# Sohojoe/ppo-dash

Measured on AMD Instinct MI355X. Metric: env-steps/sec (rollout+GAE+PPO update) at 4096 envs×128 steps, 1/2/4/8 MI355X, higher is better.
Workload: dtype f32

## Files before the change

ppo-dash_amd/csrc/conv1.hip:

```cpp
#include "conv_launch.h"
#include "conv1_fwd_body.h"
#include "conv1_paths.h"

namespace {
template <typename InT, class C_>
struct Conv1Fwd : C_ {
  using BCtx = typename C_::BCtx;
  const InT* obs; const int64_t* idx; long long row0; int C, M;
  const float* w; const float* bias; float* out;
  struct ACtx { const InT* base; bool ok; };
  __device__ ACtx a_ctx(int m, int) const {
    if (m >= M) return {obs, false};
    const int b = m / 400, pp = m - b * 400, oy = pp / 20, ox = pp - oy * 20;
    return {obs + obs_row(idx, row0, b) * (long long)(C * IMG2) + (oy * 4) * IMG + ox * 4, true};
  }
  using Raw = std::conditional_t<sizeof(InT) == 1, uint32_t, f32x4>;
  __device__ Raw a_load(const ACtx& c, int k) const {
    if (!c.ok) return Raw{};
    const int ch = k >> 6, ky = (k >> 3) & 7, kx = k & 7;
    return *reinterpret_cast<const Raw*>(c.base + ch * IMG2 + ky * IMG + kx);
  }
  __device__ BCtx b_ctx(int n, int) const { return {w + n * (C * 64), 0, n < 32}; }
  __device__ f32x4 b_load(const BCtx& c, int k) const {
    return c.ok ? *reinterpret_cast<const f32x4*>(c.p + k) : zero4();
  }
  __device__ void k_range(int, int& b, int& e) const { b = 0; e = C * 64; }
  __device__ void store(int m, int n, int, float v) const {
    if constexpr (sizeof(InT) == 1) v *= (1.0f / 255.0f);
    if (m < M) out[(size_t)m * 32 + n] = fmaxf(v + bias[n], 0.f);
  }
};

template <int C, bool MASK, int NPW = 3>
__global__ __launch_bounds__(512) void conv1_fwd_bf16x3_kernel(const uint8_t* __restrict__ obs,
                                                               const int64_t* __restrict__ idx, long long row0,
                                                               int B, const float* __restrict__ w,
                                                               const float* __restrict__ bias,
                                                               float* __restrict__ out,
                                                               uint16_t* __restrict__ mbits) {
  __shared__ __attribute__((aligned(16))) uint16_t img[2][C * C1S];
  conv1_fwd_bf16x3_body<C, MASK, NPW>(obs, idx, row0, B, w, bias, out, mbits, img);
}

template <int NPD = 3, int NW = 8, int TPW = 1>
__global__ __launch_bounds__(NW * 64) void conv1_wgrad_parts_kernel(const float* __restrict__ dz1,
                                                                const uint8_t* __restrict__ obs,
                                                                const int64_t* __restrict__ idx, long long row0,
                                                                int B, float* __restrict__ slab,
                                                                float* __restrict__ slab_bias, int dbg) {
  const bool no_mma = dbg & 1, no_put = dbg & 2, no_dma = dbg & 4;
  constexpr int C = 4, NPART = 5, ER = 20, SLOTS = 40, DZS = 88, MAXIMG = 512;
  constexpr int E_BF = C * ER * SLOTS * 4, DZ_BF = 32 * DZS, STG = E_BF + 3 * DZ_BF;
  constexpr int EPC = 105, EPIECE = 448, DPIECE = 640, RAWP = EPIECE + DPIECE;
  __shared__ __attribute__((aligned(16))) uint16_t L[2 * STG];
  __shared__ __attribute__((aligned(16))) uint4 RAW[3][RAWP];
  __shared__ long long rowtab[MAXIMG];
  __shared__ float bred[320];
  static_assert(NW == 8 || NW == 16, "8 or 16 waves");
  static_assert(TPW == 1 || (TPW == 2 && NW == 16), "two tiles per wave with 16 waves");
  constexpr int NT = NW * 64;
  const int tid = threadIdx.x, lane = tid & 63, wave = tid >> 6, l32 = lane & 31, h = lane >> 5;
  const int tile = TPW == 2 ? 2 * (wave & 3) : wave & 7, kh = TPW == 2 ? wave >> 2 : wave >> 3;
  const int G = gridDim.x;
  const int nimg = blockIdx.x < B ? (B - 1 - (int)blockIdx.x) / G + 1 : 0, nit = NPART * nimg;
  for (int k = tid; k < nimg; k += NT) rowtab[k] = obs_row(idx, row0, (int)blockIdx.x + k * G);
  int qoff[TPW][5][2];
#pragma unroll
  for (int t = 0; t < TPW; ++t) {
    const int tt = tile + t, bc = tt >> 1, bky = 4 * (tt & 1) + (l32 >> 3), bkx = l32 & 7;
#pragma unroll
    for (int ls = 0; ls < 5; ++ls)
#pragma unroll
      for (int j = 0; j < 2; ++j) {
        const int ql = 4 * ls + 2 * h + j, oyl = ql / 5, Q = ql - 5 * oyl;
        const int r = bc * ER + 4 * oyl + bky, item = r * 5 + Q;
        qoff[t][ls][j] = (r * SLOTS + Q * 8 + (bkx ^ ((item >> 1) & 7))) * 4;
      }
  }
  const int aoff = E_BF + l32 * DZS + 8 * h;
  const bool e_on = tid < 400, d_on = NW == 8 ? tid < 320 : tid >= 512 && tid < 832;
  const int eit = e_on ? tid : 0, dit = d_on ? tid - (NW == 8 ? 0 : 512) : 0;
  const int er = eit / 5, eQ = eit - 5 * er, ec = er / ER, eyr = er - ER * ec, ef = (eit >> 1) & 7;
  const int dco = dit & 31, doc = dit >> 5;
  float bacc = 0.f;
  auto dma = [&](int j) {
    if (no_dma) return;
    const int jj = j < nit ? j : nit - 1, k = jj / NPART, p = jj - NPART * k, b = (int)blockIdx.x + k * G;
    uint4* dst = RAW[jj % 3];
    if (wave < 7) {
      const int piece = min(64 * wave + lane, C * EPC - 1), c = piece / EPC, r = piece - EPC * c;
      const uint8_t* src = obs + rowtab[k] * (long long)(C * IMG2) + c * IMG2 + p * (16 * IMG) + 16 * r;
      __builtin_amdgcn_global_load_lds(reinterpret_cast<const void*>(src),
                                       reinterpret_cast<__attribute__((address_space(3))) void*>(
                                           reinterpret_cast<uintptr_t>(dst + 64 * wave)), 16, 0, 0);
    }
    const char* dsrc = reinterpret_cast<const char*>(dz1 + (size_t)b * 12800 + p * 80 * 32);
#pragma unroll
    for (int i = 0; i < (NW == 8 ? 2 : 1); ++i) {
      const int blk = NW == 8 ? wave + 8 * i : wave - 6;
      if (blk >= 0 && blk < DPIECE / 64)
        __builtin_amdgcn_global_load_lds(reinterpret_cast<const void*>(dsrc + 16 * (64 * blk + lane)),
                                         reinterpret_cast<__attribute__((address_space(3))) void*>(
                                             reinterpret_cast<uintptr_t>(dst + EPIECE + 64 * blk)), 16, 0, 0);
    }
  };
  auto put = [&](int j, int st) {
    if (no_put) return;
    const uint32_t* R = reinterpret_cast<const uint32_t*>(RAW[j % 3]);
    uint32_t ew[5];
    float dv[8];
    if (NW == 8 || e_on) {
#pragma unroll
      for (int q = 0; q < 5; ++q) ew[q] = R[(ec * 1680 + eyr * IMG + 16 * eQ) / 4 + q];
    }
    if (NW == 8 || d_on) {
#pragma unroll
      for (int q = 0; q < 8; ++q) dv[q] = __uint_as_float(R[4 * EPIECE + (8 * doc + q) * 32 + dco]);
    }
    uint16_t* S = L + st * STG;
    if (e_on) {
#pragma unroll
      for (int kx = 0; kx < 8; ++kx) {
        const int o = kx >> 2, sh = 8 * (kx & 3);
        float f[4];
// ... 115 lines not shown
#pragma unroll
      for (int t = 0; t < 2; ++t)
#pragma unroll
        for (int r = 0; r < 16; ++r) X[xo(tp, t, r)] = acc[t][r];
    }
    __syncthreads();
    if (kh == 0) {
#pragma unroll
      for (int t = 0; t < 2; ++t)
#pragma unroll
        for (int r = 0; r < 16; ++r) acc[t][r] += X[xo(tp, t, r)];
    }
  }
  float* out = slab + (size_t)blockIdx.x * 32 * 256;
  if (kh == 0) {
#pragma unroll
    for (int t = 0; t < TPW; ++t)
#pragma unroll
      for (int r = 0; r < 16; ++r) {
        const int co = (r & 3) + 8 * (r >> 2) + 4 * h, n = 32 * (tile + t) + l32;
        out[co * 256 + n] = acc[t][r];
      }
  }
  if (d_on) bred[dit] = bacc;
  __syncthreads();
  if (tid < 32) {
    float t = 0.f;
#pragma unroll
    for (int o = 0; o < 10; ++o) t += bred[32 * o + tid];
    slab_bias[(size_t)blockIdx.x * 32 + tid] = t;
  }
}

__global__ __launch_bounds__(256) void relu_bits_kernel(const float* __restrict__ a1, long long halves,
                                                        uint16_t* __restrict__ mbits) {
  for (long long i = (long long)blockIdx.x * 256 + threadIdx.x; i < halves; i += (long long)gridDim.x * 256) {
    const f32x4* p = reinterpret_cast<const f32x4*>(a1 + 16 * i);
    uint32_t m = 0;
#pragma unroll
    for (int q = 0; q < 4; ++q) {
      const f32x4 v = p[q];
#pragma unroll
      for (int e = 0; e < 4; ++e) m |= (v[e] > 0.f ? 1u : 0u) << (4 * q + e);
    }
    mbits[i] = (uint16_t)m;
  }
}

template <typename InT, class C_>
struct Conv1Wgrad : WgradBase<C_> {
  static_assert(400 % C_::BK == 0, "conv1 wgrad k-tiles must not straddle images");
  static constexpr bool B_TILE = true;
  const InT* obs; const int64_t* idx; long long row0; int C;
  struct BCtx { int off; bool ok; };
  struct TCtx { const InT* img; int r0; };
  using Raw = std::conditional_t<sizeof(InT) == 1, uint32_t, f32x4>;
  __device__ BCtx b_ctx(int n, int) const {
    const int ch = n >> 6, ky = (n >> 3) & 7, kx = n & 7;
    return {ch * IMG2 + ky * IMG + kx, n < C * 64};
  }
  __device__ TCtx tile(int k0) const {
    const int b = k0 / 400;
    return {obs + obs_row(idx, row0, b) * (long long)(C * IMG2), b * 400};
  }
  __device__ Raw b_load_t(const BCtx& c, const TCtx& t, int r) const {
    if (!c.ok || r >= this->R) return Raw{};
    const int pp = r - t.r0, oy = pp / 20, ox = pp - oy * 20;
    return *reinterpret_cast<const Raw*>(t.img + (oy * 4) * IMG + ox * 4 + c.off);
  }
};

using V32_0 = Cfg<256, 32, 4, 1, true, true>;
using CfgW32 = Cfg<32, 256, 1, 4, false, false, true>;

}

static int conv1_fwd_impl(const void* obs, int obs_is_u8, const int64_t* idx, long long row0, int C, int B,
                          const float* w1, const float* b1, float* out, uint16_t* mbits, void* stream) {
  PPO_REQUIRE(B >= 0 && C > 0, "ppo_conv1_fwd: B=%d C=%d", B, C);
  if (!mbits && B > 0 && B <= tune_small_b() && C <= 8)
    return small_conv1_fwd(obs, obs_is_u8, idx, row0, C, B, w1, b1, out, as_stream(stream));
  if (!obs_is_u8 && C == 4 && ((uintptr_t)obs & 15) == 0)
    return ppo_conv1_fwd_f32((const float*)obs, idx, row0, B, w1, b1, out, reinterpret_cast<uint32_t*>(mbits), stream);
  const bool img = obs_is_u8 && C == 4 && tune_key(TK_CONV1_FWD) == 0;
  if (mbits && !img) {
    const int rc = conv1_fwd_impl(obs, obs_is_u8, idx, row0, C, B, w1, b1, out, nullptr, stream);
    if (rc != 0 || B == 0) return rc;
    const long long halves = (long long)B * 800;
    const long long nb = (halves + 255) / 256;
    relu_bits_kernel<<<(unsigned)(nb < 8192 ? nb : 8192), 256, 0, as_stream(stream)>>>(out, halves, mbits);
    PPO_LAUNCH_CHECK("relu_bits_kernel");
    return 0;
  }
  const long long M = (long long)B * 400;
  const double fl = 2.0 * M * 32 * C * 64;
  if (img) {
    if (B == 0) return 0;
    const unsigned nb = img_grid(B);
    int slot;
    const bool prof = ppo_prof_begin("conv1_fwd_u8", as_stream(stream), &slot);
    const uint8_t* o8 = (const uint8_t*)obs;
    hipStream_t st = as_stream(stream);
    if (tune_products() == 1) {
      if (mbits) conv1_fwd_bf16x3_kernel<4, true, 1><<<nb, 512, 0, st>>>(o8, idx, row0, B, w1, b1, out, mbits);
      else conv1_fwd_bf16x3_kernel<4, false, 1><<<nb, 512, 0, st>>>(o8, idx, row0, B, w1, b1, out, nullptr);
    } else if (mbits) {
      conv1_fwd_bf16x3_kernel<4, true><<<nb, 512, 0, st>>>(o8, idx, row0, B, w1, b1, out, mbits);
    } else {
      conv1_fwd_bf16x3_kernel<4, false><<<nb, 512, 0, st>>>(o8, idx, row0, B, w1, b1, out, nullptr);
    }
    if (prof) ppo_prof_end(slot, st, fl);
    PPO_LAUNCH_CHECK("conv1_fwd_u8 (image-resident)");
    return 0;
  }
#define SETUP1(T_)                                                                                 \
  p.obs = (const T_*)obs; p.idx = idx; p.row0 = row0; p.C = C; p.M = (int)M; p.w = w1; p.bias = b1; p.out = out
  if (obs_is_u8) {
    Conv1Fwd<uint8_t, V32_0> p;
    SETUP1(uint8_t);
    return launch(p, M, 32, 1, as_stream(stream), "conv1_fwd_u8", fl);
  }
  Conv1Fwd<float, V32_0> p;
  SETUP1(float);
  return launch(p, M, 32, 1, as_stream(stream), "conv1_fwd_f32", fl);
#undef SETUP1
}

PPO_API int ppo_conv1_fwd(const void* obs, int obs_is_u8, const int64_t* idx, long long row0, int C, int B,
                          const float* w1, const float* b1, float* out, void* stream) {
  return conv1_fwd_impl(obs, obs_is_u8, idx, row0, C, B, w1, b1, out, nullptr, stream);
}

PPO_API int ppo_conv1_fwd_mask(const void* obs, int obs_is_u8, const int64_t* idx, long long row0, int C, int B,
                               const float* w1, const float* b1, float* out, uint32_t* mbits, void* stream) {
  PPO_REQUIRE(mbits != nullptr, "ppo_conv1_fwd_mask: null mask");
  return conv1_fwd_impl(obs, obs_is_u8, idx, row0, C, B, w1, b1, out, reinterpret_cast<uint16_t*>(mbits), stream);
}

PPO_API int ppo_conv1_wgrad(const float* dz1, const void* obs, int obs_is_u8, const int64_t* idx, long long row0,
                            int C, int B, int Z, float* slab, float* slab_bias, void* stream) {
  const long long R = (long long)B * 400;
  PPO_REQUIRE(R < 0x7fffffffLL, "ppo_conv1_wgrad: B too large");
  if (B <= 0 || Z <= 0) return 0;
  const double fl = 2.0 * R * 32 * C * 64;
  const int kw = tune_key(TK_CONV1_WGRAD), np = tune_products();
  if (obs_is_u8 && C == 4 && (kw == 5 || np == 1)) {
    if (B <= 0 || Z <= 0) return 0;
    PPO_REQUIRE((B + Z - 1) / Z <= 512, "ppo_conv1_wgrad: %d images over %d blocks (at most 512 per block)", B, Z);
    int slot;
    const bool prof = ppo_prof_begin("conv1_wgrad_u8", as_stream(stream), &slot);
    if (np == 1)
      conv1_wgrad_parts_kernel<1, 16, 2><<<Z, 1024, 0, as_stream(stream)>>>(dz1, (const uint8_t*)obs, idx, row0, B,
                                                                            slab, slab_bias, 0);
    else
      conv1_wgrad_parts_kernel<3, 16, 2><<<Z, 1024, 0, as_stream(stream)>>>(dz1, (const uint8_t*)obs, idx, row0, B,
                                                                            slab, slab_bias, tune_stagger() >> 4);
    if (prof) ppo_prof_end(slot, as_stream(stream), fl);
    PPO_LAUNCH_CHECK("conv1_wgrad_parts_kernel");
    return 0;
  }
  if (obs_is_u8 && C == 4)
    return kw >= 9
               ? conv1_wgrad_kw3(dz1, (const uint8_t*)obs, idx, row0, B, Z, slab, slab_bias, stream, kw == 10 ? 8 : 4)
               : conv1_wgrad_kw(dz1, (const uint8_t*)obs, idx, row0, B, Z, slab, slab_bias, stream);
  if (!obs_is_u8 && C == 4 && ((uintptr_t)obs & 15) == 0)
    return ppo_conv1_wgrad_f32(dz1, (const float*)obs, idx, row0, B, Z, slab, slab_bias, stream);
  if (obs_is_u8) {
    Conv1Wgrad<uint8_t, CfgW32> p;
    set_wgrad(p, dz1, 32, R, Z, slab, slab_bias, C * 64);
    p.obs = (const uint8_t*)obs; p.idx = idx; p.row0 = row0; p.C = C;
    return launch(p, 32, C * 64, Z, as_stream(stream), "conv1_wgrad_u8", fl);
  }
  Conv1Wgrad<float, CfgW32> p;
  set_wgrad(p, dz1, 32, R, Z, slab, slab_bias, C * 64);
  p.obs = (const float*)obs; p.idx = idx; p.row0 = row0; p.C = C;
  return launch(p, 32, C * 64, Z, as_stream(stream), "conv1_wgrad_f32", fl);
}
```

ppo-dash_amd/csrc/conv1_fwd_body.h:

```cpp
#pragma once
#include "igemm_x9.h"

namespace {

constexpr int IMG = 84, IMG2 = 84 * 84;
constexpr int C1S = 7104;
static_assert(C1S >= IMG2 && (C1S / 2) % 64 == 32, "conv1 stage channel stride");

template <int C, bool MASK, int NPW = 3>
__device__ __forceinline__ void conv1_fwd_bf16x3_body(const uint8_t* __restrict__ obs,
                                                      const int64_t* __restrict__ idx, long long row0, int B,
                                                      const float* __restrict__ w, const float* __restrict__ bias,
                                                      float* __restrict__ out, uint16_t* __restrict__ mbits,
                                                      uint16_t (*__restrict__ img)[C * C1S]) {
  constexpr int NPX = C * IMG2, CH = NPX / 16, K = C * 64, KS = K / 32, PER = (CH + 511) / 512;
  constexpr int CCH = IMG2 / 16;
  static_assert(IMG2 % 16 == 0 && C % 2 == 0, "16-pixel chunks, channel pairs");
  const int tid = threadIdx.x, lane = tid & 63, wave = tid >> 6;
  const int ct = wave & 1, rq = wave >> 1;
  const int i16 = lane & 15, g = lane >> 4;
  const int col = ct * 16 + i16;
  const float bv = bias[col];
  bf16x8 wf[3][KS];
#pragma unroll
// ... 27 lines not shown
        const uint32_t v[4] = {stage[j].x, stage[j].y, stage[j].z, stage[j].w};
        uint32_t o[8];
#pragma unroll
        for (int q = 0; q < 4; ++q) {
          const f32x4 f = to_f32x4(v[q]);
          o[2 * q] = __builtin_amdgcn_perm(__float_as_uint(f[1]), __float_as_uint(f[0]), 0x07060302u);
          o[2 * q + 1] = __builtin_amdgcn_perm(__float_as_uint(f[3]), __float_as_uint(f[2]), 0x07060302u);
        }
        const int ch = c / CCH;
        uint4* d = reinterpret_cast<uint4*>(img[buf] + ch * C1S + 16 * (c - ch * CCH));
        d[0] = uint4{o[0], o[1], o[2], o[3]};
        d[1] = uint4{o[4], o[5], o[6], o[7]};
      }
    }
  };
  const int G = gridDim.x;
  int b = blockIdx.x, cur = 0;
  if (b < B) {
    fetch(b);
    put(0);
    if (b + G < B) fetch(b + G);
  }
  __syncthreads();
  for (; b < B; b += G) {
    if (b + G < B) put(cur ^ 1);
    if (b + 2 * G < B) fetch(b + 2 * G);
    auto tiles = [&](auto ntc) __attribute__((always_inline)) {
      constexpr int NTL = decltype(ntc)::value;
      const uint16_t* I = img[cur];
      f32x4 acc[NTL];
#pragma unroll
      for (int t = 0; t < NTL; ++t) acc[t] = zero4();
      int pix[NTL];
#pragma unroll
      for (int t = 0; t < NTL; ++t) {
        const int row = (rq + 4 * t) * 16 + i16, oy = row / 20, ox = row - oy * 20;
        pix[t] = (g & 1) * C1S + (g >> 1) * IMG + oy * (4 * IMG) + ox * 4;
      }
#pragma unroll
      for (int s = 0; s < KS; ++s) {
        const uint16_t* Is = I + 2 * (s >> 2) * C1S + 2 * (s & 3) * IMG;
        bf16x8 a[NTL];
#pragma unroll
        for (int t = 0; t < NTL; ++t) {
          typedef uint32_t u32x2 __attribute__((ext_vector_type(2)));
          const volatile __attribute__((address_space(3))) u32x2* p2 =
              (const volatile __attribute__((address_space(3))) u32x2*)(Is + pix[t]);
          const u32x2 lo = p2[0], hi = p2[1];
          a[t] = __builtin_bit_cast(bf16x8, uint4{lo.x, lo.y, hi.x, hi.y});
        }
#pragma unroll
        for (int part = 0; part < NPW; ++part)
#pragma unroll
          for (int t = 0; t < NTL; ++t)
            acc[t] = __builtin_amdgcn_mfma_f32_16x16x32_bf16(a[t], wf[part][s], acc[t], 0, 0, 0);
      }
      float* o = out + (size_t)b * (400 * 32) + col;
#pragma unroll
      for (int t = 0; t < NTL; ++t) {
          const int rt = rq + 4 * t;
          uint64_t bal[4];
#pragma unroll
          for (int r = 0; r < 4; ++r) {
            const float v = fmaxf(acc[t][r] * (1.0f / 255.0f) + bv, 0.f);
            o[(rt * 16 + 4 * g + r) * 32] = v;
            if constexpr (MASK) bal[r] = __builtin_amdgcn_ballot_w64(v > 0.f);
          }
          if constexpr (MASK) {
            if (lane < 16) {
              const int r = lane & 3, gg = lane >> 2;
              const uint64_t bsel = r == 0 ? bal[0] : r == 1 ? bal[1] : r == 2 ? bal[2] : bal[3];
              mbits[((size_t)b * 400 + rt * 16 + lane) * 2 + ct] = (uint16_t)(bsel >> (16 * gg));
            }
          }
        }
    };
    if (rq == 0) tiles(std::integral_constant<int, 7>{});
    else tiles(std::integral_constant<int, 6>{});
    __syncthreads();
    cur ^= 1;
  }
}

constexpr int C1F_LDS = 2 * 4 * C1S * 2;

}
```

ppo-dash_amd/csrc/trunk.hip:

```cpp
#include "conv_launch.h"
#include "conv1_fwd_body.h"
#include "conv2_fwd_body.h"
#include "conv3_fwd_body.h"

namespace {

constexpr int max_of(int a, int b) { return a > b ? a : b; }
constexpr int TRUNK_LDS = max_of(max_of(C1F_LDS, C2F_LDS), max_of(C3C_LDS0, C3L_LDS));
static_assert(C2L_LDS <= TRUNK_LDS, "the trunk's conv2 lone tiles in the shared LDS");

__device__ __forceinline__ void trunk_phase_sync() {
  asm volatile("s_waitcnt vmcnt(0)" ::: "memory");
  __syncthreads();
  __builtin_amdgcn_fence(__ATOMIC_ACQUIRE, "agent");
}

template <int NP>
__global__ __launch_bounds__(512) void trunk_fwd_kernel(const uint8_t* __restrict__ obs, const int64_t* __restrict__ idx,
                                                       long long row0, int B, const float* __restrict__ w1,
                                                       const float* __restrict__ b1, float* __restrict__ a1,
                                                       const uint16_t* __restrict__ w2pl, const float* __restrict__ b2,
                                                       float* __restrict__ a2, const uint16_t* __restrict__ w3pl,
                                                       const float* __restrict__ b3, float* __restrict__ a3) {
  __shared__ __attribute__((aligned(16))) uint8_t lds[TRUNK_LDS];
  conv1_fwd_bf16x3_body<4, false, NP == 1 ? 1 : 3>(obs, idx, row0, B, w1, b1, a1, nullptr,
                                                   reinterpret_cast<uint16_t (*)[4 * C1S]>(lds));
  trunk_phase_sync();
  conv2_fwd_x9c_body<NP, false, true>(a1, B, w2pl, b2, a2, nullptr, lds);
  trunk_phase_sync();
  conv3_fwd_c3_body<NP, 512>(a2, B, w3pl, b3, a3, lds);
}

}

PPO_API int ppo_trunk_fwd(const uint8_t* obs, const int64_t* idx, long long row0, int B, const float* w1,
                          const float* b1, float* a1, uint32_t* m1, const float* w2p, const float* b2, float* a2,
                          uint64_t* m2, const float* w3p, const float* b3, float* a3, void* stream) {
  PPO_REQUIRE(B >= 0 && obs != nullptr && (m1 == nullptr) == (m2 == nullptr),
              "ppo_trunk_fwd: B=%d, obs and both-or-neither masks required", B);
  if (B == 0) return 0;
  if (B <= tune_small_b() || tune_key(TK_CONV1_FWD) != 0 || m1 != nullptr) {
    int rc = m1 ? ppo_conv1_fwd_mask(obs, 1, idx, row0, 4, B, w1, b1, a1, m1, stream)
                : ppo_conv1_fwd(obs, 1, idx, row0, 4, B, w1, b1, a1, stream);
    if (rc == 0)
      rc = m2 ? ppo_conv2_fwd_mask(a1, B, w2p, b2, a2, m2, stream) : ppo_conv2_fwd(a1, B, w2p, b2, a2, stream);
    if (rc == 0) rc = ppo_conv3_fwd(a2, B, w3p, b3, a3, stream);
    return rc;
  }
  const unsigned nb = img_grid(B);
  hipStream_t st = as_stream(stream);
  int slot;
  const bool prof = ppo_prof_begin("trunk_fwd", st, &slot);
  const uint16_t* w2pl = planes_of(w2p, 64 * 512);
  const uint16_t* w3pl = planes_of(w3p, 32 * 576);
  PPO_LAUNCH_NP(trunk_fwd_kernel, nb, 512, st, obs, idx, row0, B, w1, b1, a1, w2pl, b2, a2, w3pl, b3, a3);
  if (prof) ppo_prof_end(slot, st, 2.0 * B * (400.0 * 32 * 256 + 81.0 * 64 * 512 + 49.0 * 32 * 576));
  PPO_LAUNCH_CHECK("trunk_fwd_kernel");
  return 0;
}
```

ppo-dash_amd/csrc/tune.hip:

```cpp
#include "common.h"
#include "tune.h"

static const char* g_tune_names[TK_N] = {"conv1_fwd", "conv1_wgrad", "x9", "fc_splitk", "rgb_aff", "fc_splitk_tile",
                                       "conv3_dgrad_group"};
static int g_tune[TK_N] = {0, 9, 1, 4, 1, 1, 1};
static int g_stagger = 2;
static int g_small_b = 4;
static int g_split_products = 6;
static int g_heads_lds = 1;

int tune_key(int k) { return g_tune[k]; }
int tune_products() { return g_split_products; }
int tune_stagger() { return g_stagger; }
int tune_small_b() { return g_small_b; }
bool tune_heads_lds() { return g_heads_lds != 0; }

static bool tune_ok(int k, int v) {
  switch (k) {
    case TK_CONV1_FWD: return v == 0 || v == 9;
    case TK_CONV1_WGRAD: return v == 5 || v == 8 || v == 9 || v == 10;
    case TK_X9: return v >= 0 && v <= 2;
    case TK_FC_SPLITK: return v >= 0 && v <= 8;
    case TK_FC_SPLITK_TILE: return v == 0 || v == 1;
    default: return v == 0 || v == 1;
  }
}

PPO_API int ppo_tune_set(const char* key, int value) {
  if (strcmp(key, "heads_lds") == 0) {
    g_heads_lds = value;
    return 0;
  }
  if (strcmp(key, "small_b") == 0) {
    PPO_REQUIRE(value >= 0, "ppo_tune_set: small_b must be >= 0, got %d", value);
    g_small_b = value;
    return 0;
  }

  if (strcmp(key, "stagger") == 0) {
#ifndef PPO_DIAG
    PPO_REQUIRE(value >= 0 && value < 16, "ppo_tune_set: stagger takes schedule bits 0..15, got %d "
                "(the anatomy bits need a -DPPO_DIAG build)", value);
#endif
    g_stagger = value;
    return 0;
  }
  if (strcmp(key, "products") == 0) {
    PPO_REQUIRE(value == 1 || value == 6 || value == 9, "ppo_tune_set: products must be 1, 6 or 9, got %d", value);
    g_split_products = value;
    return 0;
  }
  for (int i = 0; i < TK_N; ++i)
    if (strcmp(key, g_tune_names[i]) == 0) {
      PPO_REQUIRE(tune_ok(i, value), "ppo_tune_set: %s = %d is not a kept variant", key, value);
      g_tune[i] = value;
      return 0;
    }
  ppo_set_error("ppo_tune_set: unknown key %s", key);
  return PPO_EARG;
}

PPO_API int ppo_tune_get(const char* key) {
  if (strcmp(key, "heads_lds") == 0) return g_heads_lds;
  if (strcmp(key, "small_b") == 0) return g_small_b;
  if (strcmp(key, "stagger") == 0) return g_stagger;
  if (strcmp(key, "products") == 0) return g_split_products;
  for (int i = 0; i < TK_N; ++i)
    if (strcmp(key, g_tune_names[i]) == 0) return g_tune[i];
  return -1;
}
```

ppo-dash_amd/csrc/igemm_x9.h:

```cpp
#pragma once
#include "igemm.h"
#include "tune.h"

namespace {

typedef __bf16 bf16x2 __attribute__((ext_vector_type(2)));
typedef float f32x2 __attribute__((ext_vector_type(2)));

struct Frag3 {
  bf16x8 h, m, l;
};

__device__ __forceinline__ void split8(const f32x4& x0, const f32x4& x1, Frag3& f, bool exact) {
  const float v[8] = {x0[0], x0[1], x0[2], x0[3], x1[0], x1[1], x1[2], x1[3]};
  float r[8];
#pragma unroll
  for (int j = 0; j < 8; j += 2) {
    const bf16x2 h = __builtin_convertvector(f32x2{v[j], v[j + 1]}, bf16x2);
    f.h[j] = h[0];
    f.h[j + 1] = h[1];
    r[j] = v[j] - (float)h[0];
    r[j + 1] = v[j + 1] - (float)h[1];
  }
  if (exact) return;
// ... 267 lines not shown
    if (kt + 1 < nk) gload(kbeg + (kt + 1) * BK);
    const float* As = smem + buf * STAGE;
    const float* Bs = As + SA;
    if constexpr (P::BIAS_FROM_A) {
      static_assert(NT % BM == 0 && BK % (NT / BM) == 0, "bias partials");
      constexpr int G = NT / BM;
      if (n0 == 0) {
        const int row = tid % BM;
#pragma unroll
        for (int k = (tid / BM) * 4; k < BK; k += 4 * G) {
          const f32x4 v = *reinterpret_cast<const f32x4*>(As + x9_off(row, k));
          bias_acc += (v[0] + v[1]) + (v[2] + v[3]);
        }
      }
    }
    if constexpr (BPL) {
      const uint16_t* Bp = reinterpret_cast<const uint16_t*>(Bs);
      Frag3 fa[TM];
#pragma unroll
      for (int i = 0; i < TM; ++i) frag(As, (wm * TM + i) * 16 + fr, fa[i], P::A_EXACT);
#pragma unroll
      for (int j = 0; j < TN; ++j) {
        const int row = (wn * TN + j) * 16 + fr, o = pl_off(row, fg);
        Frag3 fb;
        fb.h = *reinterpret_cast<const bf16x8*>(Bp + o);
        fb.m = *reinterpret_cast<const bf16x8*>(Bp + BN * 32 + o);
        fb.l = *reinterpret_cast<const bf16x8*>(Bp + 2 * BN * 32 + o);
#pragma unroll
        for (int i = 0; i < TM; ++i) acc[i][j] = mma9<P::A_EXACT, false, NP>(fa[i], fb, acc[i][j]);
      }
    } else {
      Frag3 fb[TN];
#pragma unroll
      for (int j = 0; j < TN; ++j) frag(Bs, (wn * TN + j) * 16 + fr, fb[j], P::B_EXACT);
#pragma unroll
      for (int i = 0; i < TM; ++i) {
        Frag3 fa;
        frag(As, (wm * TM + i) * 16 + fr, fa, P::A_EXACT);
#pragma unroll
        for (int j = 0; j < TN; ++j) acc[i][j] = mma9<P::A_EXACT, P::B_EXACT, NP>(fa, fb[j], acc[i][j]);
      }
    }
    if (kt + 1 < nk) sstore(buf ^ 1);
    __syncthreads();
  }

  bool vec_done = false;
  if constexpr (P::VEC_STORE) {
    if (p.vec) {
      vec_epilogue<P, TM, TN>(p, smem, acc, wave, lane, m0 + wm * TM * 16, n0 + wn * TN * 16, z);
      vec_done = true;
    }
  }
  if (!vec_done) {
#pragma unroll
    for (int i = 0; i < TM; ++i)
#pragma unroll
      for (int j = 0; j < TN; ++j)
#pragma unroll
        for (int r = 0; r < 4; ++r)
          p.store(m0 + (wm * TM + i) * 16 + 4 * fg + r, n0 + (wn * TN + j) * 16 + fr, z, acc[i][j][r]);
  }
  if constexpr (P::BIAS_FROM_A) {
    if (n0 == 0) {
      __syncthreads();
      constexpr int G = NT / BM;
      smem[tid] = bias_acc;
      __syncthreads();
      if (tid < BM) {
        float t = smem[tid];
#pragma unroll
        for (int g = 1; g < G; ++g) t += smem[g * BM + tid];
        p.store_bias(m0 + tid, z, t);
      }
    }
  }
}

template <int BM_, int BN_, int WM_, int WN_, bool AKC, bool BKC, bool BIASA = false, bool BP_ = false>
struct CfgS : CfgX<BM_, BN_, WM_, WN_, AKC, BKC, BIASA, false, false, BP_> {
  static constexpr bool SPLIT_STAGE = true;
};

template <class P, int NP>
__global__ __launch_bounds__(P::NT) void igemm_x9s_kernel(const P p) {
  constexpr int BM = P::BM, BN = P::BN, NT = P::NT, WM = P::WM, WN = P::WN, BK = 32;
  constexpr int TM = BM / (16 * WM), TN = BN / (16 * WN);
  static_assert(TM * 16 * WM == BM && TN * 16 * WN == BN && WM * WN * 64 == NT, "tile config");
  static_assert(!P::A_EXACT && !P::B_EXACT, "split staging: fp32 operands");
  constexpr bool BPL = P::B_PLANES, AKC = P::A_KC, BKC = P::B_KC;
  constexpr int NPL = NP == 1 ? 1 : 3;
  constexpr int PA = BM * BK, PB = BN * BK;
  constexpr int STAGE = NPL * PA + (BPL ? 3 : NPL) * PB;
  constexpr int UA = AKC ? BM * 4 : (BM / 4) * 4;
  constexpr int UB = BPL ? BN * 12 : BKC ? BN * 4 : (BN / 4) * 4;
  constexpr int NUA = (UA + NT - 1) / NT, NUB = (UB + NT - 1) / NT;
  constexpr int LA = AKC ? 2 : 8, LB = BPL ? 1 : BKC ? 2 : 8;
  constexpr int BOFF = (NT - UA % NT) % NT;
  __shared__ __attribute__((aligned(16))) uint16_t smem[2 * STAGE];
  static_assert(!P::BIAS_FROM_A || (!AKC && UA <= NT && BM * 8 <= 2 * STAGE), "bias partials: wgrad layout");

  const int tid = threadIdx.x, lane = tid & 63, wave = tid >> 6;
  const int wm = wave / WN, wn = wave % WN;
  int m0, n0, z;
  tile_of(p.n_fast, BM, BN, m0, n0, z);
  int kbeg, kend;
  p.k_range(z, kbeg, kend);
  const int nk = kend > kbeg ? (kend - kbeg + BK - 1) / BK : 0;

  typename P::ACtx actx[NUA];
  typename P::BCtx bctx[NUB];
  int ak[NUA], arow[NUA], bk[NUB], brow[NUB];
  bool aon[NUA], bon[NUB];
#pragma unroll
  for (int i = 0; i < NUA; ++i) {
    const int u = tid + i * NT;
    aon[i] = (i + 1) * NT <= UA || u < UA;
    if constexpr (AKC) {
      arow[i] = u >> 2;
      ak[i] = 8 * (u & 3);
    } else {
      arow[i] = 4 * (u % (BM / 4));
      ak[i] = 8 * (u / (BM / 4));
    }
    actx[i] = p.a_ctx(m0 + (aon[i] ? arow[i] : 0), z);
  }
#pragma unroll
  for (int i = 0; i < NUB; ++i) {
    const int u = (tid + BOFF) % NT + i * NT;
    bon[i] = (i + 1) * NT <= UB || u < UB;
    if constexpr (BPL) {
      brow[i] = (u % (BN * 4)) / 4;
      bk[i] = (u / (BN * 4)) * 4 + u % 4;
      bctx[i] = typename P::BCtx{};
      continue;
    }
    if constexpr (BKC) {
      brow[i] = u >> 2;
      bk[i] = 8 * (u & 3);
    } else {
      brow[i] = 4 * (u % (BN / 4));
      bk[i] = 8 * (u / (BN / 4));
    }
    bctx[i] = p.b_ctx(n0 + (bon[i] ? brow[i] : 0), z);
  }

  using ARaw = decltype(p.a_load(actx[0], 0));
  auto bload = [&](int i, int k) {
    if constexpr (BPL) {
      const int n = n0 + brow[i], pl = (k - (k & ~(BK - 1))) >> 2, kk = (k & ~(BK - 1)) + 8 * (k & 3);
      return bpl_load(p, n, pl, kk);
    } else {
      return p.b_load(bctx[i], k);
    }
  };
  using BRaw = decltype(bload(0, 0));
  ARaw ra[NUA][LA];
  BRaw rb[NUB][LB];
  auto gload = [&](int k0) {
#pragma unroll
    for (int i = 0; i < NUA; ++i)
#pragma unroll
      for (int j = 0; j < LA; ++j) ra[i][j] = aon[i] ? p.a_load(actx[i], k0 + ak[i] + (AKC ? 4 * j : j)) : ARaw{};
#pragma unroll
    for (int i = 0; i < NUB; ++i)
#pragma unroll
      for (int j = 0; j < LB; ++j) {
        if constexpr (BPL) rb[i][j] = bon[i] ? bload(i, k0 + bk[i]) : BRaw{};
        else rb[i][j] = bon[i] ? bload(i, k0 + bk[i] + (BKC ? 4 * j : j)) : BRaw{};
      }
  };
  float bias_acc[4] = {0.f, 0.f, 0.f, 0.f};
  auto put8 = [&](uint16_t* S, int pstride, int row, int q, const f32x4& x0, const f32x4& x1) {
    Frag3 f;
    split8(x0, x1, f, NP == 1);
    const int o = pl_off(row, q);
    *reinterpret_cast<bf16x8*>(S + o) = f.h;
    if constexpr (NPL == 3) {
      *reinterpret_cast<bf16x8*>(S + pstride + o) = f.m;
      *reinterpret_cast<bf16x8*>(S + 2 * pstride + o) = f.l;
    }
  };
  auto sstore = [&](int buf, bool bias_on) {
    uint16_t* As = smem + buf * STAGE;
    uint16_t* Bs = As + NPL * PA;
#pragma unroll
    for (int i = 0; i < NUA; ++i) {
      if (!aon[i]) continue;
      if constexpr (AKC) {
        put8(As, PA, arow[i], ak[i] >> 3, to_f32x4(ra[i][0]), to_f32x4(ra[i][1]));
      } else {
        f32x4 v[8];
#pragma unroll
        for (int j = 0; j < 8; ++j) v[j] = to_f32x4(ra[i][j]);
#pragma unroll
        for (int q = 0; q < 4; ++q) {
          const f32x4 x0 = {v[0][q], v[1][q], v[2][q], v[3][q]}, x1 = {v[4][q], v[5][q], v[6][q], v[7][q]};
          put8(As, PA, arow[i] + q, ak[i] >> 3, x0, x1);
          if constexpr (P::BIAS_FROM_A)
            if (bias_on) bias_acc[q] += ((x0[0] + x0[1]) + (x0[2] + x0[3])) + ((x1[0] + x1[1]) + (x1[2] + x1[3]));
        }
      }
    }
#pragma unroll
    for (int i = 0; i < NUB; ++i) {
      if (!bon[i]) continue;
      if constexpr (BPL) {
        *reinterpret_cast<uint4*>(Bs + (bk[i] >> 2) * PB + pl_off(brow[i], bk[i] & 3)) = rb[i][0];
      } else if constexpr (BKC) {
        put8(Bs, PB, brow[i], bk[i] >> 3, to_f32x4(rb[i][0]), to_f32x4(rb[i][1]));
      } else {
        f32x4 v[8];
#pragma unroll
        for (int j = 0; j < 8; ++j) v[j] = to_f32x4(rb[i][j]);
#pragma unroll
        for (int q = 0; q < 4; ++q)
          put8(Bs, PB, brow[i] + q, bk[i] >> 3, f32x4{v[0][q], v[1][q], v[2][q], v[3][q]},
               f32x4{v[4][q], v[5][q], v[6][q], v[7][q]});
      }
    }
  };

  f32x4 acc[TM][TN];
#pragma unroll
  for (int i = 0; i < TM; ++i)
#pragma unroll
    for (int j = 0; j < TN; ++j) acc[i][j] = zero4();

  const int fr = lane & 15, fg = lane >> 4;
  const bool bias_on = P::BIAS_FROM_A && n0 == 0;
  if (nk > 0) {
    gload(kbeg);
    sstore(0, bias_on);
  }
  __syncthreads();
  for (int kt = 0; kt < nk; ++kt) {
    const int buf = kt & 1;
    if (kt + 1 < nk) gload(kbeg + (kt + 1) * BK);
    const uint16_t* As = smem + buf * STAGE;
    const uint16_t* Bs = As + NPL * PA;
    Frag3 fb[TN];
#pragma unroll
    for (int j = 0; j < TN; ++j) {
      const int o = pl_off((wn * TN + j) * 16 + fr, fg);
      fb[j].h = *reinterpret_cast<const bf16x8*>(Bs + o);
      if constexpr (NPL == 3) {
        fb[j].m = *reinterpret_cast<const bf16x8*>(Bs + PB + o);
        fb[j].l = *reinterpret_cast<const bf16x8*>(Bs + 2 * PB + o);
      }
    }
#pragma unroll
    for (int i = 0; i < TM; ++i) {
      const int o = pl_off((wm * TM + i) * 16 + fr, fg);
      Frag3 fa;
      fa.h = *reinterpret_cast<const bf16x8*>(As + o);
      if constexpr (NPL == 3) {
        fa.m = *reinterpret_cast<const bf16x8*>(As + PA + o);
        fa.l = *reinterpret_cast<const bf16x8*>(As + 2 * PA + o);
      }
#pragma unroll
      for (int j = 0; j < TN; ++j) acc[i][j] = mma9<false, false, NP>(fa, fb[j], acc[i][j]);
    }
    if (kt + 1 < nk) sstore(buf ^ 1, bias_on);
    __syncthreads();
  }

  bool vec_done = false;
  if constexpr (P::VEC_STORE) {
    if (p.vec) {
      vec_epilogue<P, TM, TN>(p, reinterpret_cast<float*>(smem), acc, wave, lane, m0 + wm * TM * 16, n0 + wn * TN * 16,
                              z);
      vec_done = true;
    }
  }
  if (!vec_done) {
#pragma unroll
    for (int i = 0; i < TM; ++i)
#pragma unroll
      for (int j = 0; j < TN; ++j)
#pragma unroll
        for (int r = 0; r < 4; ++r)
          p.store(m0 + (wm * TM + i) * 16 + 4 * fg + r, n0 + (wn * TN + j) * 16 + fr, z, acc[i][j][r]);
  }
  if constexpr (P::BIAS_FROM_A) {
    if (bias_on) {
      __syncthreads();
      float* red = reinterpret_cast<float*>(smem);
      if (aon[0])
#pragma unroll
        for (int q = 0; q < 4; ++q) red[(ak[0] >> 3) * BM + arow[0] + q] = bias_acc[q];
      __syncthreads();
      if (tid < BM) p.store_bias(m0 + tid, z, (red[tid] + red[BM + tid]) + (red[2 * BM + tid] + red[3 * BM + tid]));
    }
  }
}

template <class P>
int launch_x9(const P& p, long long M, int N, int Z, hipStream_t st, const char* name, double flops) {
  if (M <= 0 || N <= 0 || Z <= 0) return 0;
  const long long gx = (M + P::BM - 1) / P::BM;
  if (gx > 0x7fffffffLL) {
    ppo_set_error("%s: grid too large (M=%lld)", name, M);
    return PPO_ESHAPE;
  }
  if constexpr (P::B_PLANES) {
    if (6LL * p.bps >= 0x80000000LL) {
      ppo_set_error("%s: B planes too large (%lld elements)", name, p.bps);
      return PPO_ESHAPE;
    }
  }
  dim3 grid((unsigned)gx, (unsigned)((N + P::BN - 1) / P::BN), (unsigned)Z);
  int slot;
  const bool prof = ppo_prof_begin(name, st, &slot);
  const int np = tune_products();
  if constexpr (P::SPLIT_STAGE) {
    if (np == 9) igemm_x9s_kernel<P, 9><<<grid, P::NT, 0, st>>>(p);
    else if (np == 1) igemm_x9s_kernel<P, 1><<<grid, P::NT, 0, st>>>(p);
    else igemm_x9s_kernel<P, 6><<<grid, P::NT, 0, st>>>(p);
  } else {
    if (np == 9) igemm_x9_kernel<P, 9><<<grid, P::NT, 0, st>>>(p);
    else if (np == 1) igemm_x9_kernel<P, 1><<<grid, P::NT, 0, st>>>(p);
    else igemm_x9_kernel<P, 6><<<grid, P::NT, 0, st>>>(p);
  }
  if (prof) ppo_prof_end(slot, st, flops);
  PPO_LAUNCH_CHECK(name);
  return 0;
}

}
```

ppo-dash_amd/csrc/tune.h:

```cpp
#pragma once

enum { TK_CONV1_FWD, TK_CONV1_WGRAD, TK_X9, TK_FC_SPLITK, TK_RGB_AFF, TK_FC_SPLITK_TILE,
       TK_CONV3_DGRAD_GROUP, TK_N };

int tune_key(int k);
int tune_products();
int tune_stagger();
int tune_small_b();
bool tune_heads_lds();
```

Before: 1.619 million.

## Add two-stream conv1 forward kernel with half-size blocks and single LDS image buffer

Adds a conv1 forward variant that uses 256-thread blocks, each holding one LDS image buffer instead of two. Two blocks can then be resident per CU, and the grid is sized to twice the CU count. Each block register-prefetches the next image while computing the current one, and this path becomes the default when occupancy allows two resident blocks. The trade-off is double buffering inside a block against overlap across two co-resident blocks, which brings more registers per thread and a persistent grid.

After: 1.628 million, median of 6. Within noise of the previous version (+0.6%).

```diff
diff --git a/ppo-dash_amd/csrc/conv1.hip b/ppo-dash_amd/csrc/conv1.hip
--- a/ppo-dash_amd/csrc/conv1.hip
+++ b/ppo-dash_amd/csrc/conv1.hip
@@ -31,15 +31,41 @@
   }
 };
 
-template <int C, bool MASK, int NPW = 3>
-__global__ __launch_bounds__(512) void conv1_fwd_bf16x3_kernel(const uint8_t* __restrict__ obs,
-                                                               const int64_t* __restrict__ idx, long long row0,
-                                                               int B, const float* __restrict__ w,
-                                                               const float* __restrict__ bias,
-                                                               float* __restrict__ out,
-                                                               uint16_t* __restrict__ mbits) {
-  __shared__ __attribute__((aligned(16))) uint16_t img[2][C * C1S];
-  conv1_fwd_bf16x3_body<C, MASK, NPW>(obs, idx, row0, B, w, bias, out, mbits, img);
+constexpr int C1F_DEFAULT_STREAMS = 2;
+
+template <int C, bool MASK, int NPW = 3, int STREAMS = 1>
+__global__ __launch_bounds__(512 / STREAMS, STREAMS) void conv1_fwd_bf16x3_kernel(const uint8_t* __restrict__ obs,
+                                                                                const int64_t* __restrict__ idx,
+                                                                                long long row0, int B,
+                                                                                const float* __restrict__ w,
+                                                                                const float* __restrict__ bias,
+                                                                                float* __restrict__ out,
+                                                                                uint16_t* __restrict__ mbits) {
+  static_assert(STREAMS == 1 || STREAMS == 2, "one or two image streams per CU");
+  __shared__ __attribute__((aligned(16))) uint16_t img[3 - STREAMS][C * C1S];
+  if constexpr (STREAMS == 2)
+    conv1_fwd_bf16x3_streams_body<C, MASK, NPW>(obs, idx, row0, B, w, bias, out, mbits, img[0]);
+  else
+    conv1_fwd_bf16x3_body<C, MASK, NPW>(obs, idx, row0, B, w, bias, out, mbits, img);
+}
+
+template <bool MASK, int NPW>
+static void conv1_fwd_img_launch(const uint8_t* obs, const int64_t* idx, long long row0, int B, const float* w1,
+                                 const float* b1, float* out, uint16_t* mbits, hipStream_t st) {
+  static int resident = -1;
+  if (resident < 0 && hipOccupancyMaxActiveBlocksPerMultiprocessor(&resident, conv1_fwd_bf16x3_kernel<4, MASK, NPW, 2>,
+                                                                   256, 0) != hipSuccess) {
+    (void)hipGetLastError();
+    resident = 0;
+  }
+  const int form = tune_key(TK_CONV1_FWD);
+  if ((form == 4 || (form == 0 && C1F_DEFAULT_STREAMS == 2)) && resident >= 2) {
+    const int n2 = 2 * device_cus();
+    const unsigned nb = (unsigned)(B < n2 ? B : n2);
+    conv1_fwd_bf16x3_kernel<4, MASK, NPW, 2><<<nb, 256, 0, st>>>(obs, idx, row0, B, w1, b1, out, mbits);
+  } else {
+    conv1_fwd_bf16x3_kernel<4, MASK, NPW><<<img_grid(B), 512, 0, st>>>(obs, idx, row0, B, w1, b1, out, mbits);
+  }
 }
 
 template <int NPD = 3, int NW = 8, int TPW = 1>
@@ -321,7 +347,7 @@
     return small_conv1_fwd(obs, obs_is_u8, idx, row0, C, B, w1, b1, out, as_stream(stream));
   if (!obs_is_u8 && C == 4 && ((uintptr_t)obs & 15) == 0)
     return ppo_conv1_fwd_f32((const float*)obs, idx, row0, B, w1, b1, out, reinterpret_cast<uint32_t*>(mbits), stream);
-  const bool img = obs_is_u8 && C == 4 && tune_key(TK_CONV1_FWD) == 0;
+  const bool img = obs_is_u8 && C == 4 && tune_key(TK_CONV1_FWD) != 9;
   if (mbits && !img) {
     const int rc = conv1_fwd_impl(obs, obs_is_u8, idx, row0, C, B, w1, b1, out, nullptr, stream);
     if (rc != 0 || B == 0) return rc;
@@ -335,18 +361,17 @@
   const double fl = 2.0 * M * 32 * C * 64;
   if (img) {
     if (B == 0) return 0;
-    const unsigned nb = img_grid(B);
     int slot;
     const bool prof = ppo_prof_begin("conv1_fwd_u8", as_stream(stream), &slot);
     const uint8_t* o8 = (const uint8_t*)obs;
     hipStream_t st = as_stream(stream);
     if (tune_products() == 1) {
-      if (mbits) conv1_fwd_bf16x3_kernel<4, true, 1><<<nb, 512, 0, st>>>(o8, idx, row0, B, w1, b1, out, mbits);
-      else conv1_fwd_bf16x3_kernel<4, false, 1><<<nb, 512, 0, st>>>(o8, idx, row0, B, w1, b1, out, nullptr);
+      if (mbits) conv1_fwd_img_launch<true, 1>(o8, idx, row0, B, w1, b1, out, mbits, st);
+      else conv1_fwd_img_launch<false, 1>(o8, idx, row0, B, w1, b1, out, nullptr, st);
     } else if (mbits) {
-      conv1_fwd_bf16x3_kernel<4, true><<<nb, 512, 0, st>>>(o8, idx, row0, B, w1, b1, out, mbits);
+      conv1_fwd_img_launch<true, 3>(o8, idx, row0, B, w1, b1, out, mbits, st);
     } else {
-      conv1_fwd_bf16x3_kernel<4, false><<<nb, 512, 0, st>>>(o8, idx, row0, B, w1, b1, out, nullptr);
+      conv1_fwd_img_launch<false, 3>(o8, idx, row0, B, w1, b1, out, nullptr, st);
     }
     if (prof) ppo_prof_end(slot, st, fl);
     PPO_LAUNCH_CHECK("conv1_fwd_u8 (image-resident)");
diff --git a/ppo-dash_amd/csrc/conv1_fwd_body.h b/ppo-dash_amd/csrc/conv1_fwd_body.h
--- a/ppo-dash_amd/csrc/conv1_fwd_body.h
+++ b/ppo-dash_amd/csrc/conv1_fwd_body.h
@@ -133,6 +133,128 @@
   }
 }
 
-constexpr int C1F_LDS = 2 * 4 * C1S * 2;
-
+template <int C, bool MASK, int NPW = 3>
+__device__ __forceinline__ void conv1_fwd_bf16x3_streams_body(const uint8_t* __restrict__ obs,
+                                                              const int64_t* __restrict__ idx, long long row0,
+                                                              int B, const float* __restrict__ w,
+                                                              const float* __restrict__ bias,
+                                                              float* __restrict__ out, uint16_t* __restrict__ mbits,
+                                                              uint16_t* __restrict__ img) {
+  constexpr int NPX = C * IMG2, CH = NPX / 16, K = C * 64, KS = K / 32, PER = (CH + 255) / 256;
+  constexpr int CCH = IMG2 / 16;
+  static_assert(IMG2 % 16 == 0 && C % 2 == 0, "16-pixel chunks, channel pairs");
+  const int tid = threadIdx.x, lane = tid & 63, wave = tid >> 6;
+  const int ct = wave & 1, hf = wave >> 1;
+  const int i16 = lane & 15, g = lane >> 4;
+  const int col = ct * 16 + i16;
+  const float bv = bias[col];
+  bf16x8 wf[3][KS];
+#pragma unroll
+  for (int s = 0; s < KS; ++s) {
+    const int c = 2 * (s >> 2) + (g & 1), ky = 2 * (s & 3) + (g >> 1);
+    const float* wp = w + (size_t)col * K + c * 64 + ky * 8;
+    uint32_t h[8], m[8], l[8];
+#pragma unroll
+    for (int j = 0; j < 8; ++j) split_bf16x3(wp[j], h[j], m[j], l[j]);
+#pragma unroll
+    for (int j = 0; j < 8; ++j) {
+      wf[0][s][j] = __builtin_bit_cast(__bf16, (uint16_t)h[j]);
+      wf[1][s][j] = __builtin_bit_cast(__bf16, (uint16_t)m[j]);
+      wf[2][s][j] = __builtin_bit_cast(__bf16, (uint16_t)l[j]);
+    }
+  }
+  uint4 stage[PER];
+  auto fetch = [&](int b) {
+    const uint4* src = reinterpret_cast<const uint4*>(obs + obs_row(idx, row0, b) * (long long)NPX);
+#pragma unroll
+    for (int j = 0; j < PER; ++j) {
+      const int c = tid + 256 * j;
+      if (c < CH) stage[j] = src[c];
+    }
+  };
+  auto put = [&]() {
+#pragma unroll
+    for (int j = 0; j < PER; ++j) {
+      const int c = tid + 256 * j;
+      if (c < CH) {
+        const uint32_t v[4] = {stage[j].x, stage[j].y, stage[j].z, stage[j].w};
+        uint32_t o[8];
+#pragma unroll
+        for (int q = 0; q < 4; ++q) {
+          const f32x4 f = to_f32x4(v[q]);
+          o[2 * q] = __builtin_amdgcn_perm(__float_as_uint(f[1]), __float_as_uint(f[0]), 0x07060302u);
+          o[2 * q + 1] = __builtin_amdgcn_perm(__float_as_uint(f[3]), __float_as_uint(f[2]), 0x07060302u);
+        }
+        const int ch = c / CCH;
+        uint4* d = reinterpret_cast<uint4*>(img + ch * C1S + 16 * (c - ch * CCH));
+        d[0] = uint4{o[0], o[1], o[2], o[3]};
+        d[1] = uint4{o[4], o[5], o[6], o[7]};
+      }
+    }
+  };
+  const int G = gridDim.x;
+  int b = blockIdx.x;
+  if (b < B) fetch(b);
+  for (; b < B; b += G) {
+    put();
+    __syncthreads();
+    if (b + G < B) fetch(b + G);
+    auto tiles = [&](auto ntc, int rt0) __attribute__((always_inline)) {
+      constexpr int NTL = decltype(ntc)::value;
+      f32x4 acc[NTL];
+#pragma unroll
+      for (int t = 0; t < NTL; ++t) acc[t] = zero4();
+      int pix[NTL];
+#pragma unroll
+      for (int t = 0; t < NTL; ++t) {
+        const int row = (rt0 + 2 * t) * 16 + i16, oy = row / 20, ox = row - oy * 20;
+        pix[t] = (g & 1) * C1S + (g >> 1) * IMG + oy * (4 * IMG) + ox * 4;
+      }
+#pragma unroll
+      for (int s = 0; s < KS; ++s) {
+        const uint16_t* Is = img + 2 * (s >> 2) * C1S + 2 * (s & 3) * IMG;
+        bf16x8 a[NTL];
+#pragma unroll
+        for (int t = 0; t < NTL; ++t) {
+          typedef uint32_t u32x2 __attribute__((ext_vector_type(2)));
+          const volatile __attribute__((address_space(3))) u32x2* p2 =
+              (const volatile __attribute__((address_space(3))) u32x2*)(Is + pix[t]);
+          const u32x2 lo = p2[0], hi = p2[1];
+          a[t] = __builtin_bit_cast(bf16x8, uint4{lo.x, lo.y, hi.x, hi.y});
+        }
+#pragma unroll
+        for (int part = 0; part < NPW; ++part)
+#pragma unroll
+          for (int t = 0; t < NTL; ++t)
+            acc[t] = __builtin_amdgcn_mfma_f32_16x16x32_bf16(a[t], wf[part][s], acc[t], 0, 0, 0);
+      }
+      float* o = out + (size_t)b * (400 * 32) + col;
+#pragma unroll
+      for (int t = 0; t < NTL; ++t) {
+        const int rt = rt0 + 2 * t;
+        uint64_t bal[4];
+#pragma unroll
+        for (int r = 0; r < 4; ++r) {
+          const float v = fmaxf(acc[t][r] * (1.0f / 255.0f) + bv, 0.f);
+          o[(rt * 16 + 4 * g + r) * 32] = v;
+          if constexpr (MASK) bal[r] = __builtin_amdgcn_ballot_w64(v > 0.f);
+        }
+        if constexpr (MASK) {
+          if (lane < 16) {
+            const int r = lane & 3, gg = lane >> 2;
+            const uint64_t bsel = r == 0 ? bal[0] : r == 1 ? bal[1] : r == 2 ? bal[2] : bal[3];
+            mbits[((size_t)b * 400 + rt * 16 + lane) * 2 + ct] = (uint16_t)(bsel >> (16 * gg));
+          }
+        }
+      }
+    };
+    if (hf == 0) tiles(std::integral_constant<int, 7>{}, 0);
+    else tiles(std::integral_constant<int, 6>{}, 1);
+    tiles(std::integral_constant<int, 6>{}, hf == 0 ? 14 : 13);
+    __syncthreads();
+  }
 }
+
+constexpr int C1F_LDS =2 * 4 * C1S * 2;
+
+}
diff --git a/ppo-dash_amd/csrc/trunk.hip b/ppo-dash_amd/csrc/trunk.hip
--- a/ppo-dash_amd/csrc/trunk.hip
+++ b/ppo-dash_amd/csrc/trunk.hip
@@ -39,7 +39,7 @@
   PPO_REQUIRE(B >= 0 && obs != nullptr && (m1 == nullptr) == (m2 == nullptr),
               "ppo_trunk_fwd: B=%d, obs and both-or-neither masks required", B);
   if (B == 0) return 0;
-  if (B <= tune_small_b() || tune_key(TK_CONV1_FWD) != 0 || m1 != nullptr) {
+  if (B <= tune_small_b() || tune_key(TK_CONV1_FWD) == 9 || m1 != nullptr) {
     int rc = m1 ? ppo_conv1_fwd_mask(obs, 1, idx, row0, 4, B, w1, b1, a1, m1, stream)
                 : ppo_conv1_fwd(obs, 1, idx, row0, 4, B, w1, b1, a1, stream);
     if (rc == 0)
diff --git a/ppo-dash_amd/csrc/tune.hip b/ppo-dash_amd/csrc/tune.hip
--- a/ppo-dash_amd/csrc/tune.hip
+++ b/ppo-dash_amd/csrc/tune.hip
@@ -17,7 +17,7 @@
 
 static bool tune_ok(int k, int v) {
   switch (k) {
-    case TK_CONV1_FWD: return v == 0 || v == 9;
+    case TK_CONV1_FWD: return v == 0 || v == 4 || v == 8 || v == 9;
     case TK_CONV1_WGRAD: return v == 5 || v == 8 || v == 9 || v == 10;
     case TK_X9: return v >= 0 && v <= 2;
     case TK_FC_SPLITK: return v >= 0 && v <= 8;
```

## Pipeline split-staged x9 GEMM k-loop with wave-specialized staging roles

Applied to the files above, without the earlier changes.

Adds a pipelined variant of the split-staging x9 GEMM kernel in which dedicated waves load A or B tiles two iterations ahead and interleave their LDS split-stores with the MFMA loop, using sched barriers. It is enabled by default for configs whose staging work divides evenly into waves. The aim is to hide global-load latency and LDS staging behind matrix math instead of serialising them per k-step. The cost is more registers held for in-flight data and role imbalance between waves.

New measurement: 1.583 million before, 1.605 million after (median of 6 runs). 1.01x the previous value.

```diff
diff --git a/ppo-dash_amd/csrc/igemm_x9.h b/ppo-dash_amd/csrc/igemm_x9.h
--- a/ppo-dash_amd/csrc/igemm_x9.h
+++ b/ppo-dash_amd/csrc/igemm_x9.h
@@ -373,12 +373,28 @@
   static constexpr bool SPLIT_STAGE = true;
 };
 
-template <class P, int NP>
+template <int... I, class F>
+__device__ __forceinline__ void static_for_seq(std::integer_sequence<int, I...>, F&& f) {
+  (f(std::integral_constant<int, I>{}), ...);
+}
+template <int N, class F>
+__device__ __forceinline__ void static_for(F&& f) {
+  static_for_seq(std::make_integer_sequence<int, N>{}, f);
+}
+
+template <class P>
+constexpr bool x9s_pipe_ok() {
+  constexpr int UA = (P::BM / 4) * 4, UB = (P::BN / 4) * 4;
+  return P::SPLIT_STAGE && !P::A_KC && !P::B_KC && !P::B_PLANES && UA % 64 == 0 && UB % 64 == 0 && UA + UB <= P::NT;
+}
+
+template <class P, int NP, bool PIPE = false>
 __global__ __launch_bounds__(P::NT) void igemm_x9s_kernel(const P p) {
   constexpr int BM = P::BM, BN = P::BN, NT = P::NT, WM = P::WM, WN = P::WN, BK = 32;
   constexpr int TM = BM / (16 * WM), TN = BN / (16 * WN);
   static_assert(TM * 16 * WM == BM && TN * 16 * WN == BN && WM * WN * 64 == NT, "tile config");
   static_assert(!P::A_EXACT && !P::B_EXACT, "split staging: fp32 operands");
+  static_assert(!PIPE || x9s_pipe_ok<P>(), "pipelined k loop: wave-uniform staging roles");
   constexpr bool BPL = P::B_PLANES, AKC = P::A_KC, BKC = P::B_KC;
   constexpr int NPL = NP == 1 ? 1 : 3;
   constexpr int PA = BM * BK, PB = BN * BK;
@@ -520,14 +536,7 @@
 
   const int fr = lane & 15, fg = lane >> 4;
   const bool bias_on = P::BIAS_FROM_A && n0 == 0;
-  if (nk > 0) {
-    gload(kbeg);
-    sstore(0, bias_on);
-  }
-  __syncthreads();
-  for (int kt = 0; kt < nk; ++kt) {
-    const int buf = kt & 1;
-    if (kt + 1 < nk) gload(kbeg + (kt + 1) * BK);
+  auto mfma_step = [&](int buf, auto&& after) {
     const uint16_t* As = smem + buf * STAGE;
     const uint16_t* Bs = As + NPL * PA;
     Frag3 fb[TN];
@@ -540,8 +549,8 @@
         fb[j].l = *reinterpret_cast<const bf16x8*>(Bs + 2 * PB + o);
       }
     }
-#pragma unroll
-    for (int i = 0; i < TM; ++i) {
+    static_for<TM>([&](auto ic) {
+      constexpr int i = decltype(ic)::value;
       const int o = pl_off((wm * TM + i) * 16 + fr, fg);
       Frag3 fa;
       fa.h = *reinterpret_cast<const bf16x8*>(As + o);
@@ -551,9 +560,80 @@
       }
 #pragma unroll
       for (int j = 0; j < TN; ++j) acc[i][j] = mma9<false, false, NP>(fa, fb[j], acc[i][j]);
-    }
-    if (kt + 1 < nk) sstore(buf ^ 1, bias_on);
+      after(ic);
+    });
+  };
+  if constexpr (PIPE) {
+    constexpr int WA = UA / 64, WB = UB / 64;
+    constexpr int IP = TM < 2 ? TM : 2;
+    const int wv = __builtin_amdgcn_readfirstlane(wave);
+    auto run = [&](auto role_c) {
+      constexpr int ROLE = decltype(role_c)::value;
+      f32x4 r[8];
+      auto gl = [&](int k0) {
+#pragma unroll
+        for (int j = 0; j < 8; ++j) {
+          if constexpr (ROLE == 1) r[j] = to_f32x4(p.a_load(actx[0], k0 + ak[0] + j));
+          if constexpr (ROLE == 2) r[j] = to_f32x4(bload(0, k0 + bk[0] + j));
+        }
+      };
+      auto put = [&](int buf, int q) {
+        uint16_t* As = smem + buf * STAGE;
+        const f32x4 x0 = {r[0][q], r[1][q], r[2][q], r[3][q]}, x1 = {r[4][q], r[5][q], r[6][q], r[7][q]};
+        if constexpr (ROLE == 1) {
+          put8(As, PA, arow[0] + q, ak[0] >> 3, x0, x1);
+          if constexpr (P::BIAS_FROM_A)
+            bias_acc[q] += ((x0[0] + x0[1]) + (x0[2] + x0[3])) + ((x1[0] + x1[1]) + (x1[2] + x1[3]));
+        }
+        if constexpr (ROLE == 2) put8(As + NPL * PA, PB, brow[0] + q, bk[0] >> 3, x0, x1);
+      };
+      auto step = [&](auto stg_c, auto ld_c, int kt) {
+        constexpr bool STG = decltype(stg_c)::value && ROLE != 0, LD = decltype(ld_c)::value && ROLE != 0;
+        const int buf = kt & 1;
+        mfma_step(buf, [&](auto ic) {
+          constexpr int i = decltype(ic)::value;
+          if constexpr (STG && i < IP) {
+            constexpr int Q0 = 4 * i / IP, Q1 = 4 * (i + 1) / IP;
+#pragma unroll
+            for (int q = Q0; q < Q1; ++q) put(buf ^ 1, q);
+          }
+          if constexpr (LD && i == IP - 1) {
+            __builtin_amdgcn_sched_barrier(0);
+            gl(kbeg + (kt + 2) * BK);
+            __builtin_amdgcn_sched_barrier(0);
+          }
+        });
+        __syncthreads();
+      };
+      if constexpr (ROLE != 0) {
+        if (nk > 0) {
+          gl(kbeg);
+#pragma unroll
+          for (int q = 0; q < 4; ++q) put(0, q);
+          if (nk > 1) gl(kbeg + BK);
+        }
+      }
+      __syncthreads();
+      for (int kt = 0; kt + 2 < nk; ++kt) step(std::true_type{}, std::true_type{}, kt);
+      if (nk >= 2) step(std::true_type{}, std::false_type{}, nk - 2);
+      if (nk >= 1) step(std::false_type{}, std::false_type{}, nk - 1);
+    };
+    if (wv < WA) run(std::integral_constant<int, 1>{});
+    else if (wv < WA + WB) run(std::integral_constant<int, 2>{});
+    else run(std::integral_constant<int, 0>{});
+  } else {
+    if (nk > 0) {
+      gload(kbeg);
+      sstore(0, bias_on);
+    }
     __syncthreads();
+    for (int kt = 0; kt < nk; ++kt) {
+      const int buf = kt & 1;
+      if (kt + 1 < nk) gload(kbeg + (kt + 1) * BK);
+      mfma_step(buf, [](auto) {});
+      if (kt + 1 < nk) sstore(buf ^ 1, bias_on);
+      __syncthreads();
+    }
   }
 
   bool vec_done = false;
@@ -605,6 +685,16 @@
   const bool prof = ppo_prof_begin(name, st, &slot);
   const int np = tune_products();
   if constexpr (P::SPLIT_STAGE) {
+    if constexpr (x9s_pipe_ok<P>()) {
+if (tune_wgrad_pipe()) {
+        if (np == 9) igemm_x9s_kernel<P, 9, true><<<grid, P::NT, 0, st>>>(p);
+        else if (np == 1) igemm_x9s_kernel<P, 1, true><<<grid, P::NT, 0, st>>>(p);
+        else igemm_x9s_kernel<P, 6, true><<<grid, P::NT, 0, st>>>(p);
+        if (prof) ppo_prof_end(slot, st, flops);
+        PPO_LAUNCH_CHECK(name);
+        return 0;
+      }
+    }
     if (np == 9) igemm_x9s_kernel<P, 9><<<grid, P::NT, 0, st>>>(p);
     else if (np == 1) igemm_x9s_kernel<P, 1><<<grid, P::NT, 0, st>>>(p);
     else igemm_x9s_kernel<P, 6><<<grid, P::NT, 0, st>>>(p);
diff --git a/ppo-dash_amd/csrc/tune.h b/ppo-dash_amd/csrc/tune.h
--- a/ppo-dash_amd/csrc/tune.h
+++ b/ppo-dash_amd/csrc/tune.h
@@ -1,10 +1,11 @@
 #pragma once
 
 enum { TK_CONV1_FWD, TK_CONV1_WGRAD, TK_X9, TK_FC_SPLITK, TK_RGB_AFF, TK_FC_SPLITK_TILE,
-       TK_CONV3_DGRAD_GROUP, TK_N };
+       TK_CONV3_DGRAD_GROUP, TK_WGRAD_PIPE, TK_N };
 
 int tune_key(int k);
 int tune_products();
 int tune_stagger();
 int tune_small_b();
 bool tune_heads_lds();
+bool tune_wgrad_pipe();
diff --git a/ppo-dash_amd/csrc/tune.hip b/ppo-dash_amd/csrc/tune.hip
--- a/ppo-dash_amd/csrc/tune.hip
+++ b/ppo-dash_amd/csrc/tune.hip
@@ -2,8 +2,8 @@
 #include "tune.h"
 
 static const char* g_tune_names[TK_N] = {"conv1_fwd", "conv1_wgrad", "x9", "fc_splitk", "rgb_aff", "fc_splitk_tile",
-                                       "conv3_dgrad_group"};
-static int g_tune[TK_N] = {0, 9, 1, 4, 1, 1, 1};
+                                       "conv3_dgrad_group", "wgrad_pipe"};
+static int g_tune[TK_N] = {0, 9, 1, 4, 1, 1, 1, 1};
 static int g_stagger = 2;
 static int g_small_b = 4;
 static int g_split_products = 6;
@@ -14,6 +14,7 @@
 int tune_stagger() { return g_stagger; }
 int tune_small_b() { return g_small_b; }
 bool tune_heads_lds() { return g_heads_lds != 0; }
+bool tune_wgrad_pipe() { return g_tune[TK_WGRAD_PIPE] != 0; }
 
 static bool tune_ok(int k, int v) {
   switch (k) {
```
